# ElesionKyrie/Extreme-Video-Compression-With-Prediction-Using-Pre-trainded-Diffusion-Models-

Measured on AMD Instinct MI355X. Metric: decoded frames/sec (128x128x30) at q3, higher is better.
Workload: dtype f32

## Files before the change

extreme-video-compression-with-prediction-using-pre-trainded-diffusion-models-_amd/csrc/conv_igemm.hip:

```cpp
#include <hip/hip_runtime.h>
#include <stdint.h>
#include <stdio.h>
#include "../../include/evc_hip.h"

typedef float f32x16 __attribute__((ext_vector_type(16)));
typedef __attribute__((address_space(3))) void lds_void;
typedef const __attribute__((address_space(1))) void glb_void;

#ifndef EVC_CONV_TAIL
#define EVC_CONV_TAIL 1
#endif
#ifndef EVC_CONV_TM1
#define EVC_CONV_TM1 1
#endif
#ifndef EVC_SPLIT_WIDE_TILES
#define EVC_SPLIT_WIDE_TILES 1
#endif

#ifndef EVC_SPLIT_INTERLEAVE
#define EVC_SPLIT_INTERLEAVE 5
#endif

namespace {

constexpr int BM_MAX = 128;
constexpr int KC = 16;

constexpr int MODE_PLAIN = 0, MODE_AFFINE = 1, MODE_AFFINE_SILU = 2, MODE_SILU = 3, MODE_RELU = 4;

struct ConvK {
    const float* src0; const float* src1; int C0; int C1; int ld0; int ld1;
    const float* coef_a; const float* coef_s;
    const float* w; const float* bias; const float* res; int ld_res;
    float out_scale; int act_out;
    float* out; int ld_out;
    int B, H, W, Co, CoPad, KH, KW;
    int M, HW, nchunk, nsteps, steps_per_split, splits;
    float* ws;
    float* stats;
    const float* w_hdr;
    const unsigned* in_bound;
    int tail_first, tail_splits, tail_sps, tail_rows;
    int cut_chunk;
    const float* x2_src0; const float* x2_src1; int x2_C0, x2_C1, x2_ld0, x2_ld1;
    const char* x2_w;
    const float* x2_hdr;
    const unsigned* x2_bound;
};

__device__ __forceinline__ float in_scale(const ConvK& p) {
    if (!p.in_bound) return 1.0f;
    const float b = sqrtf(__uint_as_float(*p.in_bound));
    if (!(b < 3.0e38f)) return __builtin_nanf("");
    return b > 0.f ? ldexpf(1.0f, 6 - ilogbf(b)) : 1.0f;
}

__device__ __forceinline__ float silu_f(float v) { return v * __builtin_amdgcn_rcpf(1.0f + __expf(-v)); }

__device__ __forceinline__ float act_fn(float v, int act) {
    if (act == EVC_ACT_SILU) return silu_f(v);
    if (act == EVC_ACT_RELU) return v < 0.f ? 0.f : v;
    return v;
}

template <int MODE>
__device__ __forceinline__ float4 transform(float4 v, const float4& a, const float4& s, bool ok) {
    if (MODE == MODE_AFFINE || MODE == MODE_AFFINE_SILU) {
        v.x = v.x * a.x + s.x; v.y = v.y * a.y + s.y; v.z = v.z * a.z + s.z; v.w = v.w * a.w + s.w;
    }
    if (MODE == MODE_AFFINE_SILU || MODE == MODE_SILU) {
        v.x = silu_f(v.x); v.y = silu_f(v.y); v.z = silu_f(v.z); v.w = silu_f(v.w);
    }
    if (MODE == MODE_RELU) {
        v.x = v.x < 0.f ? 0.f : v.x; v.y = v.y < 0.f ? 0.f : v.y; v.z = v.z < 0.f ? 0.f : v.z; v.w = v.w < 0.f ? 0.f : v.w;
    }
    v.x = ok ? v.x : 0.f; v.y = ok ? v.y : 0.f; v.z = ok ? v.z : 0.f; v.w = ok ? v.w : 0.f;
    return v;
}

template <int TM, int TN>
__device__ __forceinline__ void mfma_group(f32x16 (&acc)[TM][TN], const float4 (&a)[TM], const float4 (&b)[TN]) {
#define EVC_MFMA_E(e)                                                                                   \
    _Pragma("unroll") for (int i = 0; i < TM; ++i) _Pragma("unroll") for (int j = 0; j < TN; ++j)      \
        acc[i][j] = __builtin_amdgcn_mfma_f32_32x32x2f32(a[i].e, b[j].e, acc[i][j], 0, 0, 0);
    EVC_MFMA_E(x) EVC_MFMA_E(y) EVC_MFMA_E(z) EVC_MFMA_E(w)
#undef EVC_MFMA_E
}

template <int TM, int TN, int WM, bool PARTIAL, bool RES, bool STATS, bool ACT>
__device__ __forceinline__ void conv_epilogue_full(const ConvK& p, f32x16 (&acc)[TM][TN], int m0, int n0, int split,
                                                   int wm, int wn, int l31, int half, bool tail) {
    constexpr int BM = 32 * TM * WM;
    const int ws_m0 = tail ? p.tail_first * BM : 0;
    const size_t ws_M = tail ? (size_t)p.tail_rows : (size_t)p.M;
    const float ascale = p.w_hdr ? p.w_hdr[0] / in_scale(p) : 1.0f;
    const float oscale = p.out_scale;
    const int mw = m0 + wm * 32 * TM + 4 * half;
    const int cw = n0 + wn * 32 * TN + l31;
    const bool has_res = RES && (!ACT || p.res != nullptr), has_stats = STATS && (!ACT || p.stats != nullptr);
#pragma unroll
// ... 921 lines not shown
    if (nmac > 0) {
        chunk_setup();
        load_coefs();
        load_a();
        dma_w(0);
        store_a(0);
        if (1 < nst) advance_w();
    }
    __syncthreads();

    int wb = 0, sidx = 0;

    for (int g = 0; g < nmac; ++g) {
        const int ab = g & 1;
        {
            EVC_RR_NEXT_W()
            __builtin_amdgcn_sched_barrier(0);
            if (g + 1 < nmac) advance_l();
            load_a();
            __builtin_amdgcn_sched_barrier(0);
            EVC_RR_FRAGS(0)
            EVC_RR_TERMS(0, SP::NTERM)
            __builtin_amdgcn_sched_barrier(0);
            asm volatile("s_waitcnt vmcnt(2) lgkmcnt(0)\n\ts_barrier" ::: "memory");
            __builtin_amdgcn_sched_barrier(0);
            wb ^= 1; ++sidx;
        }
        {
            EVC_RR_NEXT_W()
            EVC_RR_FRAGS(1)
            EVC_RR_TERMS(0, SP::NTERM)
            __syncthreads();
            wb ^= 1; ++sidx;
        }
        {
            EVC_RR_NEXT_W()
            __builtin_amdgcn_sched_barrier(0);
            EVC_RR_FRAGS(2)
            EVC_RR_TERMS(0, SP::NTERM / 2)
            __builtin_amdgcn_sched_barrier(0);
            store_a(ab ^ 1);
            __builtin_amdgcn_sched_barrier(0);
            EVC_RR_TERMS(SP::NTERM / 2, SP::NTERM)
            __builtin_amdgcn_sched_barrier(0);
            __syncthreads();
            wb ^= 1; ++sidx;
        }
    }
#undef EVC_RR_TERMS
#undef EVC_RR_FRAGS
#undef EVC_RR_NEXT_W

    conv_epilogue<TM, TN, WM>(p, acc, m0, n0, split, wm, wn, l31, half, tail);
}

template <bool PARTIAL, bool RES, bool STATS, bool ACT>
__device__ __forceinline__ void wide_epilogue_t(const ConvK& p, f32x16 (&acc)[4][3], char* lds, int m0, int n0, int split,
                                                int wave, int lane, bool tail) {
    constexpr int TM = 4, TN = 3, BM = 256, RS = 36;
    const int wm = wave >> 1, wn = wave & 1;
    const int l31 = lane & 31, half = lane >> 5;
    const int ws_m0 = tail ? p.tail_first * BM : 0;
    const size_t ws_M = tail ? (size_t)p.tail_rows : (size_t)p.M;
    const float ascale = p.w_hdr[0] / in_scale(p);
    const float oscale = p.out_scale;
    const bool has_res = RES && (!ACT || p.res != nullptr), has_stats = STATS && (!ACT || p.stats != nullptr);
    float* const patch0 = reinterpret_cast<float*>(lds) + wave * 2 * 32 * RS;
    const int wr = lane >> 3, wc = (lane & 7) * 4;
    const int mw = m0 + wm * 32 * TM;
    const int prow = 4 * half * RS + l31;
    constexpr int RD = 4;
    float4 rq[RD][4];
    const auto res_load = [&](int t, float4 (&dst)[4]) {
        const int jj = t / TM, ii = t - jj * TM;
        const float* rp = p.res + (size_t)(mw + ii * 32 + wr) * p.ld_res + n0 + wn * 32 * TN + jj * 32 + wc;
#pragma unroll
        for (int k = 0; k < 4; ++k) dst[k] = *reinterpret_cast<const float4*>(rp + (size_t)(8 * k) * p.ld_res);
    };
    if (has_res) {
#pragma unroll
        for (int t = 0; t < RD - 1; ++t) res_load(t, rq[t]);
    }
#pragma unroll
    for (int j = 0; j < TN; ++j) {
        const int cj = n0 + wn * 32 * TN + j * 32;
        const float bias = (!PARTIAL && p.bias) ? p.bias[cj + l31] : 0.f;
        float4 ssum = make_float4(0.f, 0.f, 0.f, 0.f), ssq = make_float4(0.f, 0.f, 0.f, 0.f);
#pragma unroll
        for (int i = 0; i < TM; ++i) {
            const int mb = mw + i * 32;
            const int tt = j * TM + i;
            if (has_res && tt + RD - 1 < TM * TN) res_load(tt + RD - 1, rq[(tt + RD - 1) % RD]);
            float* const P = patch0 + ((i * TN + j) & 1) * 32 * RS;
#pragma unroll
            for (int r = 0; r < 16; ++r) P[prow + ((r & 3) + 8 * (r >> 2)) * RS] = acc[i][j][r] * ascale + bias;
#pragma unroll
            for (int k = 0; k < 4; ++k) {
                float4 q = *reinterpret_cast<const float4*>(P + (wr + 8 * k) * RS + wc);
                const int m = mb + wr + 8 * k;
                if (!PARTIAL) {
                    if (has_res) { const float4& rr = rq[tt % RD][k]; q.x += rr.x; q.y += rr.y; q.z += rr.z; q.w += rr.w; }
                    q.x *= oscale; q.y *= oscale; q.z *= oscale; q.w *= oscale;
                    if (ACT) { q.x = act_fn(q.x, p.act_out); q.y = act_fn(q.y, p.act_out); q.z = act_fn(q.z, p.act_out); q.w = act_fn(q.w, p.act_out); }
                    if (STATS) {
                        ssum.x += q.x; ssum.y += q.y; ssum.z += q.z; ssum.w += q.w;
                        ssq.x += q.x * q.x; ssq.y += q.y * q.y; ssq.z += q.z * q.z; ssq.w += q.w * q.w;
// ... 571 lines not shown

extern "C" long long evc_conv_packed_bytes(int Co, int Ci, int KH, int KW, int arith) {
    const long long elems = evc_conv_packed_floats(Co, Ci, KH, KW);
    switch (arith) {
        case EVC_ARITH_F32: return elems * 4;
        case EVC_ARITH_BF16X6: return elems * 6;
        case EVC_ARITH_F16X3: return F16_HDR_BYTES + elems * 4;
        default: return EVC_EINVAL;
    }
}

extern "C" int evc_conv_pack_weights(const float* w, void* packed, int Co, int Ci, int KH, int KW, int arith,
                                     void* stream) {
    if (arith == EVC_ARITH_F32) return evc_conv_pack_weights_f32(w, (float*)packed, Co, Ci, KH, KW, stream);
    if (arith != EVC_ARITH_BF16X6 && arith != EVC_ARITH_F16X3) return EVC_EINVAL;
    if (!w || !packed || Co <= 0 || Ci <= 0 || Ci % KC != 0 || KH <= 0 || KW <= 0) return EVC_EINVAL;
    const long long total = evc_conv_packed_floats(Co, Ci, KH, KW);
    int grid = (int)((total + 255) / 256 > 4096 ? 4096 : (total + 255) / 256);
    hipStream_t st = (hipStream_t)stream;
    if (arith == EVC_ARITH_BF16X6) {
        hipLaunchKernelGGL(conv_pack_split_kernel, dim3(grid), dim3(256), 0, st, w, (__bf16*)packed, Co,
                           evc_conv_co_pad(Co), Ci, KH, KW);
    } else {
        if (hipMemsetAsync(packed, 0, F16_HDR_BYTES, st) != hipSuccess) return EVC_ELAUNCH;
        const size_t n = (size_t)Co * Ci * KH * KW;
        hipLaunchKernelGGL(conv_absmax_kernel, dim3(grid), dim3(256), 0, st, w, n, reinterpret_cast<unsigned*>(packed) + 2);
        hipLaunchKernelGGL(conv_pack_f16_kernel, dim3(grid), dim3(256), 0, st, w, (char*)packed, Co,
                           evc_conv_co_pad(Co), Ci, KH, KW);
    }
    return hipGetLastError() == hipSuccess ? EVC_OK : EVC_ELAUNCH;
}

static int conv_validate(const evc_conv_args* a) {
    if (!a || !a->src0 || !a->w_packed || !a->out) return EVC_EINVAL;
    if (a->C0 <= 0 || a->C0 % KC != 0 || a->C1 < 0 || a->C1 % KC != 0) return EVC_EINVAL;
    if (a->C1 > 0 && !a->src1) return EVC_EINVAL;
    if ((a->ld0 != 0 && (a->ld0 < a->C0 || (a->ld0 & 3))) || (a->ld1 != 0 && (a->ld1 < a->C1 || (a->ld1 & 3))))
        return EVC_EINVAL;
    if ((a->coef_a == nullptr) != (a->coef_s == nullptr)) return EVC_EINVAL;
    if (a->B <= 0 || a->H <= 0 || a->W <= 0 || a->Co <= 0) return EVC_EINVAL;
    if (a->KH <= 0 || a->KW <= 0 || !(a->KH & 1) || !(a->KW & 1)) return EVC_EINVAL;
    if (a->ld_out < a->Co || (a->res && a->ld_res < a->Co)) return EVC_EINVAL;
    if ((long long)a->B * a->H * a->W > 0x7fffffffLL) return EVC_EINVAL;
    if (a->arith != EVC_ARITH_F32 && a->arith != EVC_ARITH_BF16X6 && a->arith != EVC_ARITH_F16X3) return EVC_EINVAL;
    if (a->x2_w_packed) {
        if (!a->x2_src0 || !a->x2_bound || a->x2_C0 <= 0 || a->x2_C0 % KC != 0 || a->x2_C1 < 0 || a->x2_C1 % KC != 0) return EVC_EINVAL;
        if (a->x2_C1 > 0 && !a->x2_src1) return EVC_EINVAL;
        if ((a->x2_ld0 != 0 && (a->x2_ld0 < a->x2_C0 || (a->x2_ld0 & 3))) || (a->x2_ld1 != 0 && (a->x2_ld1 < a->x2_C1 || (a->x2_ld1 & 3))))
            return EVC_EINVAL;
    }
    return EVC_OK;
}

struct TileCfg { int tm, tn, bm, bn; long long tiles; int splits; int reuse; int wide; int steps_per_split;
                 int tail_first, tail_tiles, tail_splits, tail_sps;
                 int cut_chunk; };
static int g_wide_cut = 1;
static int g_tail_split = EVC_CONV_TAIL;
static int g_wide_tiles = EVC_SPLIT_WIDE_TILES;
static int g_no_reuse = 0;
static int g_wide_mid = 1;
static int g_wide256 = 1;
static int g_force_tm = 0;

static void split_tile_cfg(const evc_conv_args* a, long long M, long long ntile, int nsteps, TileCfg& c, bool rr_ok) {
    const double K = (double)a->KH * a->KW * (a->C0 + a->C1);
    const bool f16 = a->arith == EVC_ARITH_F16X3 && rr_ok;
    const double E = f16 ? 20.0 : 6.0, F2 = f16 ? 1.5 : 1.0;
    const auto grid_time = [&](long long n, double sps) {
        const long long R = n / 512, rem = n - R * 512;
        return (sps + E) * ((double)R * F2 + (rem == 0 ? 0.0 : (rem <= 256 && f16 ? 1.0 : F2)));
    };
    double best = 1e300;
    int best_tm = 2, best_s = 1;
    c.tail_first = 0; c.tail_tiles = 0; c.tail_splits = 1; c.tail_sps = 0;
    for (int tm = 2; tm >= 1; --tm) {
        if (g_force_tm && tm != g_force_tm) continue;
        const long long tiles = ((M + 64 * tm - 1) / (64 * tm)) * ntile;
        const int smax = a->splits > 0 ? a->splits : (nsteps / 4 < 1 ? 1 : (nsteps / 4 > 32 ? 32 : nsteps / 4));
        for (int s = a->splits > 0 ? a->splits : 1; s <= smax; ++s) {
            const double sps = (double)((nsteps + s - 1) / s);
            const double slab_mb = (double)s * (double)M * a->Co * 4.0 / 1e6;
            const double pen = s > 1 ? 1.0 + (slab_mb > 192.0 ? 300.0 : 40.0) * s / K : 1.0;
            const double tmf = tm == 1 ? (a->KH * a->KW > 1 ? 0.5 / (rr_ok ? 0.55 : 0.75) : 0.5) : 1.0;
            const double t = grid_time(tiles * s, sps) * pen * tmf;
            if (t < best * 0.9999) { best = t; best_tm = tm; best_s = s; }
        }
    }
    c.tm = best_tm;
    c.bm = 64 * c.tm;
    c.tiles = ((M + c.bm - 1) / c.bm) * ntile;
    c.splits = best_s;
    if (rr_ok && g_tail_split && a->splits <= 0 && !g_force_tm && M % 128 == 0) {
        const long long tm_all = M / 128, wgs = tm_all * ntile;
        const long long R = wgs / 512;
        const long long main_m = R * 512 / ntile, tail_m = tm_all - main_m;
        const int unit = 3 * 9;
        if (R >= 1 && tail_m > 0 && nsteps >= 2 * unit) {
            int ts = (int)(512 / (tail_m * ntile));
            if (ts > nsteps / unit) ts = nsteps / unit;
            if (ts >= 2) {
                int sps = (nsteps + ts - 1) / ts;
                sps = (sps + 2) / 3 * 3;
                ts = (nsteps + sps - 1) / sps;
                const double t_tail = grid_time(main_m * ntile, (double)nsteps) +
                                      grid_time(tail_m * ntile * ts, (double)sps) * (1.0 + 40.0 * ts / K);
                if (ts >= 2 && t_tail < best * 0.98) {
                    c.tm = 2; c.bm = 128; c.tiles = wgs; c.splits = 1;
                    c.tail_first = (int)main_m; c.tail_tiles = (int)tail_m; c.tail_splits = ts; c.tail_sps = sps;
                }
            }
        }
    }
}

static inline bool is_split_arith(int arith) { return arith == EVC_ARITH_BF16X6 || arith == EVC_ARITH_F16X3; }
static inline int arith_planes(int arith) { return arith == EVC_ARITH_F16X3 ? 2 : 3; }
constexpr long long LDS_CAP = 160 * 1024;

static long long rr_lds_bytes(int np, int bm, int W, int bn) {
    return (long long)np * 32 * (2LL * (bm / W) * (W + 2) + 2LL * bn);
}

static long long wide_lds_bytes(int W, bool x2) { return (x2 ? 6LL : 4LL) * (256 / W + 2) * (W + 2) * 32; }

static bool wide_ok(const evc_conv_args* a) {
    const bool mode_ok = a->coef_a ? a->act_in == EVC_ACT_SILU : a->act_in == EVC_ACT_NONE;
    return g_wide256 && mode_ok && a->arith == EVC_ARITH_F16X3 && a->KH == 3 && a->KW == 3 && a->Co % 192 == 0 &&
           (a->W == 16 || a->W == 32 || a->W == 64 || a->W == 128) && ((long long)a->H * a->W) % 256 == 0 &&
           a->ld_out % 4 == 0 && (!a->res || a->ld_res % 4 == 0);
}

static TileCfg conv_tile_cfg(const evc_conv_args* a) {
    TileCfg c;
    c.wide = 0;
    c.cut_chunk = 0;
    const long long M = (long long)a->B * a->H * a->W;
    const int CoPad = evc_conv_co_pad(a->Co);
    c.tn = pick_tn(CoPad);
    c.bn = 64 * c.tn;
    const long long ntile = CoPad / c.bn;
    const int nsteps = a->KH * a->KW * ((a->C0 + a->C1) / KC);
    c.reuse = 0;
    if (is_split_arith(a->arith)) {
        const int np = arith_planes(a->arith);
        const bool rr_ok = !g_no_reuse && a->KH == 3 && a->KW == 3 && a->W >= 4 && 128 % a->W == 0 &&
                           rr_lds_bytes(np, 128, a->W, c.bn) <= LDS_CAP;
        split_tile_cfg(a, M, ntile, nsteps, c, rr_ok);
        if (rr_ok && c.tm == 2) c.reuse = 1;
        if (c.reuse && c.splits == 1 && !c.tail_tiles && g_wide_tiles && M % 256 == 0 && rr_lds_bytes(np, 256, a->W, c.bn) <= LDS_CAP) {
            const long long t256 = (M / 256) * ntile;
            if ((t256 >= 512 && t256 % 256 == 0) || t256 >= 6 * 256) {
                c.bm = 256;
                c.tiles = t256;
            }
        }
    } else {
        c.tail_first = 0; c.tail_tiles = 0; c.tail_splits = 1; c.tail_sps = 0;
        c.tm = (!EVC_CONV_TM1 || ((M + 127) / 128) * ntile >= 64) ? 2 : 1;
        if (g_force_tm) c.tm = g_force_tm;
        c.bm = 64 * c.tm;
        c.tiles = ((M + c.bm - 1) / c.bm) * ntile;
        long long splits = 1;
        if (a->splits > 0) splits = a->splits;
        else if (c.tiles < 384) {
            splits = (640 + c.tiles / 2) / c.tiles;
            const int max_by_steps = nsteps / 8 > 0 ? nsteps / 8 : 1;
            if (splits > max_by_steps) splits = max_by_steps;
            if (splits > 32) splits = 32;
            if (splits < 1) splits = 1;
        }
        c.splits = (int)splits;
    }
    if (wide_ok(a) && a->splits <= 0 && !g_force_tm) {
        const long long tm_all = M / 256, nt = a->Co / 192, wgs = tm_all * nt;
        if (wgs >= 256) {
            const int nchunk = (a->C0 + a->C1) / KC;
            c.wide = 1; c.reuse = 0; c.tm = 4; c.tn = 3; c.bm = 256; c.bn = 192; c.tiles = wgs; c.splits = 1;
            c.tail_first = 0; c.tail_tiles = 0; c.tail_splits = 1; c.tail_sps = 0;
            const long long Rr = wgs / 256;
            const long long main_m = Rr * 256 / nt, tail_m = tm_all - main_m;
            if (g_tail_split && tail_m > 0) {
                int ts = (int)(256 / (tail_m * nt));
                if (ts > nchunk / 3) ts = nchunk / 3;
                if (ts >= 2) {
                    const int cps = (nchunk + ts - 1) / ts;
                    ts = (nchunk + cps - 1) / cps;
                    c.tail_first = (int)main_m; c.tail_tiles = (int)tail_m; c.tail_splits = ts; c.tail_sps = cps * 9;
                }
            }
            c.steps_per_split = nsteps;
            return c;
        }
        if (g_wide_mid && wgs >= 32) {
            const int nchunk = (a->C0 + a->C1) / KC;
            int best_s = 0;
            double best_t = 1e300;
            for (int sp = 1; sp <= 8 && wgs * sp <= 256 && nchunk / sp >= 4; ++sp) {
                const int cps = (nchunk + sp - 1) / sp;
                const double slab_mb = sp > 1 ? (double)sp * M * a->Co * 4.0 / 1e6 : 0.0;
                const double t = 23000.0 + 13900.0 * cps + (sp > 1 ? 2.0 * 2000.0 * (5.0 + slab_mb / 4.0) : 0.0);
                if (t < best_t) { best_t = t; best_s = sp; }
            }
            if (best_s > 0 && wgs * best_s >= 128) {
                const int cps = (nchunk + best_s - 1) / best_s;
                c.wide = 1; c.reuse = 0; c.tm = 4; c.tn = 3; c.bm = 256; c.bn = 192; c.tiles = wgs;
                c.tail_first = 0; c.tail_tiles = 0; c.tail_splits = 1; c.tail_sps = 0;
                c.splits = (nchunk + cps - 1) / cps;
                c.steps_per_split = cps * 9;
                if (g_wide_cut && best_s == 1 && wgs > 128 && nchunk >= 6) {
                    const long long idle = 256 - wgs, r = (wgs + idle - 1) / idle;
                    const double slab_mb = 2.0 * M * a->Co * 4.0 / 1e6;
                    const double comb = 2.0 * 2000.0 * (5.0 + slab_mb / 4.0);
                    int cut = 0;
                    double t_cut = best_t * 0.95;
                    for (int sh = 1; sh <= nchunk / 2; ++sh) {
                        const double tl = 23000.0 + 13900.0 * (nchunk - sh), ts = (double)r * (23000.0 + 13900.0 * sh);
                        const double t = (tl > ts ? tl : ts) + comb;
                        if (t < t_cut) { t_cut = t; cut = nchunk - sh; }
                    }
                    if (cut > 0) { c.splits = 2; c.cut_chunk = cut; c.steps_per_split = cut * 9; }
                }
                return c;
            }
        }
    }
    const int unit = c.reuse ? a->KW : 1;
    int sps = (nsteps + c.splits - 1) / c.splits;
    sps = (sps + unit - 1) / unit * unit;
    c.steps_per_split = sps;
    c.splits = (nsteps + sps - 1) / sps;
    return c;
}

extern "C" int evc_conv_set_option(const char* name, int value) {
    if (!name) return EVC_EINVAL;
    const auto is = [&](const char* s) { int i = 0; while (s[i] && s[i] == name[i]) ++i; return s[i] == 0 && name[i] == 0; };
    if (is("wide_tiles")) { g_wide_tiles = value; return EVC_OK; }
    if (is("row_reuse")) { g_no_reuse = !value; return EVC_OK; }
    if (is("tail_split")) { g_tail_split = value; return EVC_OK; }
    if (is("wide256")) { g_wide256 = value; return EVC_OK; }
    if (is("wide_mid")) { g_wide_mid = value; return EVC_OK; }
    if (is("wide_cut")) { g_wide_cut = value; return EVC_OK; }
    return EVC_EINVAL;
}

extern "C" int evc_conv_fused_1x1_supported(const evc_conv_args* a) {
    if (conv_validate(a) != EVC_OK) return 0;
    if (a->arith != EVC_ARITH_F16X3 || a->KH != 3 || a->KW != 3) return 0;
    const TileCfg c = conv_tile_cfg(a);
    return (c.reuse == 1 || c.wide) ? 1 : 0;
}

extern "C" int evc_conv_kernel_name(const evc_conv_args* a, char* buf, int n) {
    if (!buf || n <= 0 || conv_validate(a) != EVC_OK) return EVC_EINVAL;
    int mode;
    if (a->coef_a) mode = a->act_in == EVC_ACT_SILU ? MODE_AFFINE_SILU : MODE_AFFINE;
    else mode = a->act_in == EVC_ACT_SILU ? MODE_SILU : a->act_in == EVC_ACT_RELU ? MODE_RELU : MODE_PLAIN;
    const TileCfg c = conv_tile_cfg(a);
    int len;
    if (c.wide) len = snprintf(buf, n, "conv_wide_kernel<%d, %d, %s>", mode, a->W == 128 ? 4 : 3, a->x2_w_packed ? "true" : "false");
    else if (is_split_arith(a->arith)) {
        const int np = arith_planes(a->arith);
        if (c.reuse) len = snprintf(buf, n, "conv_split_rr_kernel<%d, %d, %d, %d>", np, c.bm == 256 ? 4 : 2, c.tn, mode);
        else if (np == 3) len = snprintf(buf, n, "conv_split_kernel<%d, %d, %d>", c.tm, c.tn, mode);
        else len = snprintf(buf, n, "conv_splitn_kernel<2, %d, %d, %d>", c.tm, c.tn, mode);
    } else len = snprintf(buf, n, "conv_igemm_kernel<%d, %d, %d>", c.tm, c.tn, mode);
    return len;
}

extern "C" int evc_conv_choose_splits(const evc_conv_args* a) {
    if (conv_validate(a) != EVC_OK) return EVC_EINVAL;
    return conv_tile_cfg(a).splits;
}

extern "C" int evc_conv_stats_splits(const evc_conv_args* a) {
    if (conv_validate(a) != EVC_OK) return 0;
    const int HW = a->H * a->W;
    if (HW % 64 != 0) return 0;
    const TileCfg c = conv_tile_cfg(a);
    if (c.splits > 1 || c.wide) return HW / 64;
    const long long M = (long long)a->B * HW;
    const int CoPad = evc_conv_co_pad(a->Co);
    if (M % c.bm != 0 || a->Co != CoPad || a->Co % c.bn != 0) return 0;
    return HW / (32 * c.tm);
}

extern "C" long long evc_conv_workspace_bytes(const evc_conv_args* a) {
    if (conv_validate(a) != EVC_OK) return EVC_EINVAL;
    const TileCfg c = conv_tile_cfg(a);
    if (c.tail_tiles) return (long long)c.tail_splits * c.tail_tiles * c.bm * a->Co * (long long)sizeof(float);
    if (c.splits == 1) return 0;
    return (long long)c.splits * a->B * a->H * a->W * a->Co * (long long)sizeof(float);
}

static int ensure_dynamic_lds(const void* fn, unsigned long long* done_mask, size_t lds) {
    if (lds <= 64 * 1024) return EVC_OK;
    if ((long long)lds > LDS_CAP) return EVC_EUNSUPPORTED;
    int dev = 0;
    if (hipGetDevice(&dev) != hipSuccess) return EVC_ELAUNCH;
    const unsigned long long bit = 1ULL << (dev & 63);
    if (__atomic_load_n(done_mask, __ATOMIC_ACQUIRE) & bit) return EVC_OK;
    if (hipFuncSetAttribute(fn, hipFuncAttributeMaxDynamicSharedMemorySize, (int)LDS_CAP) != hipSuccess) return EVC_ELAUNCH;
    __atomic_fetch_or(done_mask, bit, __ATOMIC_RELEASE);
    return EVC_OK;
}

#ifdef EVC_DEV_FAST
#define EVC_MODE_SWITCH(mode, CALL) CALL(MODE_AFFINE_SILU);
#else
#define EVC_MODE_SWITCH(mode, CALL)                                   \
    switch (mode) {                                                   \
        case MODE_AFFINE: CALL(MODE_AFFINE); break;                   \
        case MODE_AFFINE_SILU: CALL(MODE_AFFINE_SILU); break;         \
// ... 15 lines not shown
static int launch_split3(int mode, dim3 grid, size_t lds, hipStream_t st, const ConvK& k) {
#define EVC_CALL(M) hipLaunchKernelGGL((conv_split_kernel<TM, TN, M>), grid, dim3(256), lds, st, k)
    EVC_MODE_SWITCH(mode, EVC_CALL)
#undef EVC_CALL
    return EVC_OK;
}

template <int TM, int TN>
static int launch_split2(int mode, dim3 grid, size_t lds, hipStream_t st, const ConvK& k) {
#define EVC_CALL(M) hipLaunchKernelGGL((conv_splitn_kernel<2, TM, TN, M>), grid, dim3(256), lds, st, k)
    EVC_MODE_SWITCH(mode, EVC_CALL)
#undef EVC_CALL
    return EVC_OK;
}

template <int NP, int WM, int TN, int MODE>
static int launch_split_rr_one(dim3 grid, size_t lds, hipStream_t st, const ConvK& k) {
    static unsigned long long attr_done = 0;
    const int rc = ensure_dynamic_lds(reinterpret_cast<const void*>(&conv_split_rr_kernel<NP, WM, TN, MODE>), &attr_done, lds);
    if (rc != EVC_OK) return rc;
    hipLaunchKernelGGL((conv_split_rr_kernel<NP, WM, TN, MODE>), grid, dim3(128 * WM), lds, st, k);
    return EVC_OK;
}
template <int NP, int WM, int TN>
static int launch_split_rr(int mode, dim3 grid, size_t lds, hipStream_t st, const ConvK& k) {
    int rc = EVC_OK;
#define EVC_CALL(M) rc = launch_split_rr_one<NP, WM, TN, M>(grid, lds, st, k)
    EVC_MODE_SWITCH(mode, EVC_CALL)
#undef EVC_CALL
    return rc;
}

template <int MODE, int NU, bool X2>
static int launch_wide_one(dim3 grid, size_t lds, hipStream_t st, const ConvK& k) {
    static unsigned long long attr_done = 0;
    const int rc = ensure_dynamic_lds(reinterpret_cast<const void*>(&conv_wide_kernel<MODE, NU, X2>), &attr_done, lds);
    if (rc != EVC_OK) return rc;
    hipLaunchKernelGGL((conv_wide_kernel<MODE, NU, X2>), grid, dim3(256), lds, st, k);
    return EVC_OK;
}
template <int MODE>
static int launch_wide_mode(int nu, bool x2, dim3 grid, size_t lds, hipStream_t st, const ConvK& k) {
    if (nu == 4) return x2 ? launch_wide_one<MODE, 4, true>(grid, lds, st, k) : launch_wide_one<MODE, 4, false>(grid, lds, st, k);
    return x2 ? launch_wide_one<MODE, 3, true>(grid, lds, st, k) : launch_wide_one<MODE, 3, false>(grid, lds, st, k);
}
static int launch_wide(int mode, int nu, bool x2, dim3 grid, size_t lds, hipStream_t st, const ConvK& k) {
#ifdef EVC_DEV_FAST
    return launch_wide_mode<MODE_AFFINE_SILU>(nu, x2, grid, lds, st, k);
#else
    if (mode == MODE_AFFINE_SILU) return launch_wide_mode<MODE_AFFINE_SILU>(nu, x2, grid, lds, st, k);
    if (mode == MODE_PLAIN) return launch_wide_mode<MODE_PLAIN>(nu, x2, grid, lds, st, k);
    return EVC_EUNSUPPORTED;
#endif
}

#define EVC_TN_SWITCH(tn, CALL) ((tn) == 3 ? CALL(3) : (tn) == 2 ? CALL(2) : CALL(1))

static int conv2d_impl(const evc_conv_args* a, float* ws, void* stream, hipEvent_t ev_start, hipEvent_t ev_conv_end);

extern "C" int evc_conv2d_nhwc_f32(const evc_conv_args* a, float* ws, void* stream) {
    return conv2d_impl(a, ws, stream, nullptr, nullptr);
}

extern "C" int evc_conv2d_nhwc_profiled_f32(const evc_conv_args* a, float* ws, void* stream, void* ev_start,
                                            void* ev_conv_end) {
    return conv2d_impl(a, ws, stream, (hipEvent_t)ev_start, (hipEvent_t)ev_conv_end);
}

static int conv2d_impl(const evc_conv_args* a, float* ws, void* stream, hipEvent_t ev_start, hipEvent_t ev_conv_end) {
    int rc = conv_validate(a);
    if (rc != EVC_OK) return rc;
    int mode;
    if (a->coef_a) {
        if (a->act_in == EVC_ACT_SILU) mode = MODE_AFFINE_SILU;
        else if (a->act_in == EVC_ACT_NONE) mode = MODE_AFFINE;
        else return EVC_EUNSUPPORTED;
    } else {
        mode = a->act_in == EVC_ACT_SILU ? MODE_SILU : a->act_in == EVC_ACT_RELU ? MODE_RELU : MODE_PLAIN;
        if (a->act_in != EVC_ACT_NONE && a->act_in != EVC_ACT_SILU && a->act_in != EVC_ACT_RELU) return EVC_EINVAL;
    }
    ConvK k;
    k.src0 = a->src0; k.src1 = a->src1 ? a->src1 : a->src0; k.C0 = a->C0; k.C1 = a->C1;
    k.ld0 = a->ld0 > 0 ? a->ld0 : a->C0; k.ld1 = a->ld1 > 0 ? a->ld1 : (a->C1 > 0 ? a->C1 : k.ld0);
    k.coef_a = a->coef_a; k.coef_s = a->coef_s;
    k.w = a->w_packed; k.bias = a->bias; k.res = a->res; k.ld_res = a->ld_res;
    k.w_hdr = nullptr;
    k.in_bound = nullptr;
    if (a->in_bound) {
        if (a->arith != EVC_ARITH_F16X3) return EVC_EINVAL;
        k.in_bound = a->in_bound;
    }
    if (a->arith == EVC_ARITH_F16X3) {
        k.w_hdr = a->w_packed;
        k.w = reinterpret_cast<const float*>(reinterpret_cast<const char*>(a->w_packed) + F16_HDR_BYTES);
    }
    k.out_scale = a->out_scale; k.act_out = a->act_out; k.out = a->out; k.ld_out = a->ld_out;
    k.B = a->B; k.H = a->H; k.W = a->W; k.Co = a->Co; k.CoPad = evc_conv_co_pad(a->Co);
    k.KH = a->KH; k.KW = a->KW;
    k.M = a->B * a->H * a->W; k.HW = a->H * a->W;
    if ((long long)k.M * k.ld0 * 4 >= (1LL << 32) || (long long)k.M * k.ld1 * 4 >= (1LL << 32)) return EVC_EUNSUPPORTED;
    if (a->KH * a->KW > 32) return EVC_EUNSUPPORTED;
    k.nchunk = (a->C0 + a->C1) / KC;
    k.nsteps = a->KH * a->KW * k.nchunk;
    const TileCfg cfg = conv_tile_cfg(a);
    k.splits = cfg.splits;
    k.steps_per_split = cfg.steps_per_split;
    k.ws = ws;
    if ((k.splits > 1 || cfg.tail_tiles) && !ws) return EVC_EINVAL;
    k.stats = k.splits > 1 ? nullptr : a->stats_out;
    if (a->stats_out && evc_conv_stats_splits(a) == 0) return EVC_EINVAL;
    k.x2_w = nullptr; k.x2_hdr = nullptr; k.x2_bound = nullptr; k.x2_src0 = k.x2_src1 = nullptr;
    k.x2_C0 = k.x2_C1 = k.x2_ld0 = k.x2_ld1 = 0;
    if (a->x2_w_packed) {
        if (a->arith != EVC_ARITH_F16X3 || a->KH != 3 || a->KW != 3 || !(cfg.reuse == 1 || cfg.wide)) return EVC_EUNSUPPORTED;
        k.x2_src0 = a->x2_src0; k.x2_src1 = a->x2_src1 ? a->x2_src1 : a->x2_src0;
        k.x2_C0 = a->x2_C0; k.x2_C1 = a->x2_C1;
        k.x2_ld0 = a->x2_ld0 > 0 ? a->x2_ld0 : a->x2_C0;
        k.x2_ld1 = a->x2_ld1 > 0 ? a->x2_ld1 : (a->x2_C1 > 0 ? a->x2_C1 : k.x2_ld0);
        if ((long long)k.M * k.x2_ld0 * 4 >= (1LL << 32) || (long long)k.M * k.x2_ld1 * 4 >= (1LL << 32)) return EVC_EUNSUPPORTED;
        k.x2_hdr = a->x2_w_packed;
        k.x2_w = reinterpret_cast<const char*>(a->x2_w_packed) + F16_HDR_BYTES;
        k.x2_bound = a->x2_bound;
    }
    k.tail_first = 0x7fffffff; k.tail_splits = 1; k.tail_sps = 0; k.tail_rows = 0;
    k.cut_chunk = cfg.wide ? cfg.cut_chunk : 0;
    if (cfg.tail_tiles) {
        k.tail_first = cfg.tail_first; k.tail_splits = cfg.tail_splits; k.tail_sps = cfg.tail_sps;
        k.tail_rows = cfg.tail_tiles * cfg.bm;
    }

    dim3 grid((k.M + cfg.bm - 1) / cfg.bm, k.CoPad / cfg.bn, k.splits);
    if (cfg.tail_tiles) grid.x = cfg.tail_first + cfg.tail_tiles * cfg.tail_splits;
    hipStream_t st = (hipStream_t)stream;
    if (ev_start && hipEventRecord(ev_start, st) != hipSuccess) return EVC_ELAUNCH;
    if (cfg.wide) {
        rc = launch_wide(mode, a->W == 128 ? 4 : 3, a->x2_w_packed != nullptr, grid, (size_t)wide_lds_bytes(a->W, a->x2_w_packed != nullptr), st, k);
    } else if (is_split_arith(a->arith)) {
        const int np = arith_planes(a->arith);
        if (cfg.reuse) {
            const size_t lds_rr = (size_t)rr_lds_bytes(np, cfg.bm, a->W, cfg.bn);
#define EVC_RR4_3(TN) launch_split_rr<3, 4, TN>(mode, grid, lds_rr, st, k)
#define EVC_RR2_3(TN) launch_split_rr<3, 2, TN>(mode, grid, lds_rr, st, k)
#define EVC_RR4_2(TN) launch_split_rr<2, 4, TN>(mode, grid, lds_rr, st, k)
#define EVC_RR2_2(TN) launch_split_rr<2, 2, TN>(mode, grid, lds_rr, st, k)
            if (np == 3) rc = cfg.bm == 256 ? EVC_TN_SWITCH(cfg.tn, EVC_RR4_3) : EVC_TN_SWITCH(cfg.tn, EVC_RR2_3);
            else rc = cfg.bm == 256 ? EVC_TN_SWITCH(cfg.tn, EVC_RR4_2) : EVC_TN_SWITCH(cfg.tn, EVC_RR2_2);
#undef EVC_RR4_3
#undef EVC_RR2_3
#undef EVC_RR4_2
#undef EVC_RR2_2
        } else {
            const size_t lds = (size_t)2 * np * (cfg.bm + cfg.bn) * 32;
#define EVC_S3_2(TN) launch_split3<2, TN>(mode, grid, lds, st, k)
#define EVC_S3_1(TN) launch_split3<1, TN>(mode, grid, lds, st, k)
#define EVC_S2_2(TN) launch_split2<2, TN>(mode, grid, lds, st, k)
#define EVC_S2_1(TN) launch_split2<1, TN>(mode, grid, lds, st, k)
            if (np == 3) rc = cfg.tm == 2 ? EVC_TN_SWITCH(cfg.tn, EVC_S3_2) : EVC_TN_SWITCH(cfg.tn, EVC_S3_1);
            else rc = cfg.tm == 2 ? EVC_TN_SWITCH(cfg.tn, EVC_S2_2) : EVC_TN_SWITCH(cfg.tn, EVC_S2_1);
#undef EVC_S3_2
#undef EVC_S3_1
#undef EVC_S2_2
#undef EVC_S2_1
        }
    } else {
        const size_t lds = (size_t)2 * (cfg.bm + cfg.bn) * KC * sizeof(float);
#define EVC_F_2(TN) launch_mode<2, TN>(mode, grid, lds, st, k)
#define EVC_F_1(TN) launch_mode<1, TN>(mode, grid, lds, st, k)
        rc = cfg.tm == 2 ? EVC_TN_SWITCH(cfg.tn, EVC_F_2) : EVC_TN_SWITCH(cfg.tn, EVC_F_1);
#undef EVC_F_2
#undef EVC_F_1
    }
    if (rc != EVC_OK) return rc;
    if (hipGetLastError() != hipSuccess) return EVC_ELAUNCH;
    if (ev_conv_end && hipEventRecord(ev_conv_end, st) != hipSuccess) return EVC_ELAUNCH;
    if (k.splits > 1) {
        hipLaunchKernelGGL(conv_splitk_reduce_kernel, dim3((k.M + 63) / 64, (k.Co + 63) / 64), dim3(1024), 0, st, ws,
                           k.splits, k.M, k.Co, a->bias, a->res, a->ld_res, a->out_scale, a->act_out, a->out,
                           a->ld_out, a->stats_out);
        if (hipGetLastError() != hipSuccess) return EVC_ELAUNCH;
    }
    if (cfg.tail_tiles) {
        const size_t m0 = (size_t)cfg.tail_first * cfg.bm;
        hipLaunchKernelGGL(conv_splitk_reduce_kernel, dim3((k.tail_rows + 63) / 64, (k.Co + 63) / 64), dim3(1024), 0, st, ws,
                           k.tail_splits, k.tail_rows, k.Co, a->bias, a->res ? a->res + m0 * a->ld_res : nullptr, a->ld_res,
                           a->out_scale, a->act_out, a->out + m0 * a->ld_out, a->ld_out,
                           a->stats_out ? a->stats_out + (m0 / 64) * k.Co * 2 : nullptr);
        if (hipGetLastError() != hipSuccess) return EVC_ELAUNCH;
    }
    return EVC_OK;
// ... 2 lines not shown
```

Measured before the change: 37.22.

## Add weight-stationary split-K conv kernel for small-spatial 3x3 f16x3 layers

Adds a new conv_ws_kernel for 3x3 convolutions on small images (W of 8 or 16, M up to 2304) with many input channels. Each block covers a variable number of pixels and 64 output channels. It stages the input rows in LDS once per chunk and reuses them across the three horizontal taps, and it splits K across many blocks that write partial sums to the workspace. The goal is better parallelism and less input re-fetching than the reuse tile path on these low-occupancy layers. The cost is more workspace traffic, a heuristic split selection, and four template instantiations per mode.

Result: slower. 36.62 (-1.6%).

```diff
diff --git a/extreme-video-compression-with-prediction-using-pre-trainded-diffusion-models-_amd/csrc/conv_igemm.hip b/extreme-video-compression-with-prediction-using-pre-trainded-diffusion-models-_amd/csrc/conv_igemm.hip
--- a/extreme-video-compression-with-prediction-using-pre-trainded-diffusion-models-_amd/csrc/conv_igemm.hip
+++ b/extreme-video-compression-with-prediction-using-pre-trainded-diffusion-models-_amd/csrc/conv_igemm.hip
@@ -46,6 +46,7 @@
     const char* x2_w;
     const float* x2_hdr;
     const unsigned* x2_bound;
+    int ws_pb;
 };
 
 __device__ __forceinline__ float in_scale(const ConvK& p) {
@@ -1073,6 +1074,274 @@
 #undef EVC_RR_NEXT_W
 
     conv_epilogue<TM, TN, WM>(p, acc, m0, n0, split, wm, wn, l31, half, tail);
+}
+
+constexpr int WS_NT = 512;
+constexpr int WS_NI = 5;
+constexpr int WS_NJ = 3;
+constexpr int WS_PB_MAX = 128 * WS_NI;
+constexpr int WS_PATCH = 32 * 36 * 4;
+
+template <int MODE, bool X2, int NTI>
+__device__ __forceinline__ void conv_ws_body(const ConvK& p, char* smem_b) {
+    typedef Split<2> SP;
+    typedef f16x8 vec;
+    constexpr int RB = 32;
+    constexpr int WBUF = 3 * 2 * 64 * RB;
+    constexpr bool HAS_COEF = MODE == MODE_AFFINE || MODE == MODE_AFFINE_SILU;
+    const int PB = p.ws_pb;
+    const int m0 = blockIdx.x * PB;
+    const int pbc = min(PB, p.M - m0);
+    const int nt32 = pbc >> 5;
+    const int SR = (PB / p.W) * (p.W + 2);
+    const int APL = SR * RB;
+    char* const As = smem_b;
+    char* const Ws = smem_b + 4 * APL;
+
+    const int tid = threadIdx.x;
+    const int lane = tid & 63;
+    const int wave = __builtin_amdgcn_readfirstlane(tid >> 6);
+    const int wm = wave >> 1, wn = wave & 1;
+    const int l31 = lane & 31, half = lane >> 5;
+    const int n0 = blockIdx.y * 64;
+    const int split = blockIdx.z;
+    const int Ct = p.C0 + p.C1;
+    const int kh = tid & 1;
+
+    int it_m[WS_NJ], it_lds[WS_NJ], it_b[WS_NJ];
+    unsigned it_ok[WS_NJ];
+#pragma unroll
+    for (int j = 0; j < WS_NJ; ++j) {
+        const int pl = (tid + WS_NT * j) >> 1;
+        const bool valid = pl < pbc;
+        const int plc = valid ? pl : 0;
+        const int mm = m0 + plc;
+        const int b = mm / p.HW;
+        const int y = (mm - b * p.HW) / p.W;
+        it_m[j] = mm; it_b[j] = b;
+        unsigned ok = valid ? 8u : 0u;
+#pragma unroll
+        for (int ty = 0; ty < 3; ++ty) ok |= ((valid && y + ty - 1 >= 0 && y + ty - 1 < p.H) ? 1u : 0u) << ty;
+        it_ok[j] = ok;
+        const int srow = plc + 2 * (plc / p.W) + 1;
+        it_lds[j] = srow * RB + 16 * (kh ^ ((srow >> 3) & 1));
+    }
+    int abase[NTI];
+#pragma unroll
+    for (int i = 0; i < NTI; ++i) {
+        const int t = wm + 4 * i;
+        const int ml = (t < nt32 ? t : 0) * 32 + l31;
+        abase[i] = ml + 2 * (ml / p.W);
+    }
+    const int w_rd = (wn * 32 + l31) * RB + 16 * (half ^ ((l31 >> 3) & 1));
+
+    const unsigned slab = 2u * (unsigned)p.CoPad * RB;
+    const unsigned w_tap = (unsigned)p.nchunk * slab;
+    const unsigned wsrc = (unsigned)((((wave >> 1) & 1) * p.CoPad + n0 + (wave & 1) * 32) * RB + lane * 16);
+    const int tx_a = wave >> 2;
+    const int wdst_a = ((tx_a * 2 + ((wave >> 1) & 1)) * 64 + (wave & 1) * 32) * RB;
+    const int wdst_b = ((2 * 2 + ((wave >> 1) & 1)) * 64 + (wave & 1) * 32) * RB;
+
+    const int units = p.nchunk * 3;
+    const int ups = p.steps_per_split / 3;
+    const int u_begin = split * ups;
+    const int nmac = max(0, min(units, u_begin + ups) - u_begin);
+    int n2 = 0, c2_begin = 0;
+    float s2 = 1.0f;
+    if (X2) {
+        const int nch2 = (p.x2_C0 + p.x2_C1) / KC;
+        const int per = (nch2 + p.splits - 1) / p.splits;
+        c2_begin = min(nch2, split * per);
+        n2 = min(nch2, c2_begin + per) - c2_begin;
+        const float b = sqrtf(__uint_as_float(*p.x2_bound));
+        if (!(b < 3.0e38f)) s2 = __builtin_nanf("");
+        else if (b > 0.f) s2 = ldexpf(1.0f, 6 - ilogbf(b));
+    }
+    const int total = n2 + nmac;
+    const float xscale = F16_ACT_SCALE * in_scale(p);
+    const float xscale2 = F16_ACT_SCALE * s2;
+
+    float4 areg[WS_NJ][2], ca[WS_NJ][2], cs[WS_NJ][2];
+    auto issue_x2 = [&](int s) {
+        char* wl = Ws + (s & 1) * WBUF;
+        {
+            const int c = c2_begin + s;
+            if (wave >= 4)
+                __builtin_amdgcn_global_load_lds((glb_void*)(p.x2_w + (unsigned)c * slab + wsrc), (lds_void*)(wl + wdst_a), 16, 0, 0);
+            const int cc = c * KC;
+            const bool first = cc < p.x2_C0;
+            const char* src = reinterpret_cast<const char*>(first ? p.x2_src0 : p.x2_src1);
+            const unsigned ld = (unsigned)(first ? p.x2_ld0 : p.x2_ld1);
+            const unsigned co = (unsigned)(first ? cc : cc - p.x2_C0) + 8u * kh;
+#pragma unroll
+            for (int j = 0; j < WS_NJ; ++j) {
+                const unsigned o = ((unsigned)it_m[j] * ld + co) * 4u;
+                areg[j][0] = *reinterpret_cast<const float4*>(src + o);
+                areg[j][1] = *reinterpret_cast<const float4*>(src + o + 16);
+            }
+        }
+    };
+    auto issue = [&](int s) {
+        char* wl = Ws + (s & 1) * WBUF;
+        {
+            const int u = u_begin + (s - n2);
+            const int chunk = u / 3, ty = u - chunk * 3;
+            const char* wt = reinterpret_cast<const char*>(p.w) + (unsigned)(ty * 3 * p.nchunk + chunk) * slab + wsrc;
+            __builtin_amdgcn_global_load_lds((glb_void*)(wt + (unsigned)tx_a * w_tap), (lds_void*)(wl + wdst_a), 16, 0, 0);
+            if (wave < 4)
+                __builtin_amdgcn_global_load_lds((glb_void*)(wt + 2u * w_tap), (lds_void*)(wl + wdst_b), 16, 0, 0);
+            const int c = chunk * KC;
+            const bool first = c < p.C0;
+            const char* src = reinterpret_cast<const char*>(first ? p.src0 : p.src1);
+            const unsigned ld = (unsigned)(first ? p.ld0 : p.ld1);
+            const unsigned co = (unsigned)(first ? c : c - p.C0) + 8u * kh;
+            if (HAS_COEF && (ty == 0 || s == n2)) {
+#pragma unroll
+                for (int j = 0; j < WS_NJ; ++j) {
+                    const size_t o = (size_t)it_b[j] * Ct + c + 8 * kh;
+                    ca[j][0] = *reinterpret_cast<const float4*>(p.coef_a + o);
+                    ca[j][1] = *reinterpret_cast<const float4*>(p.coef_a + o + 4);
+                    cs[j][0] = *reinterpret_cast<const float4*>(p.coef_s + o);
+                    cs[j][1] = *reinterpret_cast<const float4*>(p.coef_s + o + 4);
+                }
+            }
+#pragma unroll
+            for (int j = 0; j < WS_NJ; ++j) {
+                const bool ok = (it_ok[j] >> ty) & 1u;
+                const unsigned o = ((unsigned)(it_m[j] + (ok ? (ty - 1) * p.W : 0)) * ld + co) * 4u;
+                areg[j][0] = *reinterpret_cast<const float4*>(src + o);
+                areg[j][1] = *reinterpret_cast<const float4*>(src + o + 16);
+            }
+        }
+    };
+    auto commit_x2 = [&](int s) {
+        char* A = As + (s & 1) * 2 * APL;
+#pragma unroll
+        for (int j = 0; j < WS_NJ; ++j) {
+            if (!(it_ok[j] & 8u)) continue;
+            vec pl[2];
+            SP::split(areg[j][0], areg[j][1], xscale2, pl);
+            *reinterpret_cast<vec*>(A + it_lds[j]) = pl[0];
+            *reinterpret_cast<vec*>(A + APL + it_lds[j]) = pl[1];
+        }
+    };
+    auto commit = [&](int s) {
+        char* A = As + (s & 1) * 2 * APL;
+        const int u = u_begin + (s - n2);
+        const int ty = u - (u / 3) * 3;
+#pragma unroll
+        for (int j = 0; j < WS_NJ; ++j) {
+            if (!(it_ok[j] & 8u)) continue;
+            vec pl[2];
+            const bool ok = (it_ok[j] >> ty) & 1u;
+            SP::split(transform<MODE>(areg[j][0], ca[j][0], cs[j][0], ok), transform<MODE>(areg[j][1], ca[j][1], cs[j][1], ok), xscale, pl);
+            *reinterpret_cast<vec*>(A + it_lds[j]) = pl[0];
+            *reinterpret_cast<vec*>(A + APL + it_lds[j]) = pl[1];
+        }
+    };
+
+    f32x16 acc[NTI];
+#pragma unroll
+    for (int i = 0; i < NTI; ++i)
+#pragma unroll
+        for (int r = 0; r < 16; ++r) acc[i][r] = 0.f;
+
+    auto tap = [&](int s, int tx) {
+        const char* Ab = As + (s & 1) * 2 * APL;
+        const char* Wb = Ws + (s & 1) * WBUF + tx * (2 * 64 * RB) + w_rd;
+        vec b[2];
+        b[0] = *reinterpret_cast<const vec*>(Wb);
+        b[1] = *reinterpret_cast<const vec*>(Wb + 64 * RB);
+#pragma unroll
+        for (int i0 = 0; i0 < NTI; i0 += 2) {
+            constexpr int NPAIR = 2;
+            vec a[NPAIR][2];
+#pragma unroll
+            for (int d = 0; d < NPAIR; ++d) {
+                if (i0 + d < NTI) {
+                    const int sr = abase[i0 + d] + tx;
+                    const int o = sr * RB + 16 * (half ^ ((sr >> 3) & 1));
+                    a[d][0] = *reinterpret_cast<const vec*>(Ab + o);
+                    a[d][1] = *reinterpret_cast<const vec*>(Ab + APL + o);
+                }
+            }
+#pragma unroll
+            for (int t = 0; t < SP::NTERM; ++t)
+#pragma unroll
+                for (int d = 0; d < NPAIR; ++d)
+                    if (i0 + d < NTI) acc[i0 + d] = SP::mfma(a[d][SP::qa(t)], b[SP::qb(t)], acc[i0 + d]);
+        }
+    };
+
+    for (int o = tid * 16; o < 4 * APL; o += WS_NT * 16) *reinterpret_cast<float4*>(As + o) = make_float4(0.f, 0.f, 0.f, 0.f);
+    __syncthreads();
+    if (X2 && n2 > 0) { issue_x2(0); commit_x2(0); }
+    else if (nmac > 0) { issue(n2); commit(n2); }
+    asm volatile("s_waitcnt vmcnt(0)" ::: "memory");
+    __syncthreads();
+
+    if (X2) {
+        for (int s = 0; s < n2; ++s) {
+            const bool nx = s + 1 < n2, nm = !nx && nmac > 0;
+            if (nx) issue_x2(s + 1);
+            else if (nm) issue(s + 1);
+            tap(s, 1);
+            if (nx) commit_x2(s + 1);
+            else if (nm) commit(s + 1);
+            asm volatile("s_waitcnt vmcnt(0)" ::: "memory");
+            __syncthreads();
+        }
+        if (n2 > 0) {
+            const float r = (p.x2_hdr[0] / s2) / (p.w_hdr[0] / in_scale(p));
+#pragma unroll
+            for (int i = 0; i < NTI; ++i)
+#pragma unroll
+                for (int e = 0; e < 16; ++e) acc[i][e] *= r;
+        }
+    }
+    for (int s = n2; s < total; ++s) {
+        if (s + 1 < total) issue(s + 1);
+        tap(s, 0);
+        if (s + 1 < total) commit(s + 1);
+        tap(s, 1);
+        tap(s, 2);
+        asm volatile("s_waitcnt vmcnt(0)" ::: "memory");
+        __syncthreads();
+    }
+
+    const float ascale = p.w_hdr[0] / in_scale(p);
+    float* const patch = reinterpret_cast<float*>(smem_b + wave * WS_PATCH);
+#pragma unroll
+    for (int i = 0; i < NTI; ++i) {
+        const int t = wm + 4 * i;
+        if (t >= nt32) break;
+#pragma unroll
+        for (int r = 0; r < 16; ++r) patch[((r & 3) + 8 * (r >> 2) + 4 * half) * 36 + l31] = acc[i][r] * ascale;
+        __builtin_amdgcn_fence(__ATOMIC_RELEASE, "wavefront");
+        __builtin_amdgcn_wave_barrier();
+        __builtin_amdgcn_fence(__ATOMIC_ACQUIRE, "wavefront");
+        float* o = p.ws + ((size_t)split * p.M + (m0 + t * 32)) * p.Co + n0 + wn * 32;
+#pragma unroll
+        for (int k = 0; k < 4; ++k) {
+            const int row = (lane >> 3) + 8 * k, c4 = (lane & 7) * 4;
+            *reinterpret_cast<float4*>(o + (size_t)row * p.Co + c4) = *reinterpret_cast<const float4*>(patch + row * 36 + c4);
+        }
+        __builtin_amdgcn_fence(__ATOMIC_RELEASE, "wavefront");
+        __builtin_amdgcn_wave_barrier();
+        __builtin_amdgcn_fence(__ATOMIC_ACQUIRE, "wavefront");
+    }
+}
+
+template <int MODE, bool X2>
+__global__ __launch_bounds__(WS_NT, 1) void conv_ws_kernel(ConvK p) {
+    extern __shared__ __attribute__((aligned(16))) char smem_b[];
+    const int wm = __builtin_amdgcn_readfirstlane((int)threadIdx.x >> 7);
+    const int nt32 = min(p.ws_pb, p.M - (int)blockIdx.x * p.ws_pb) >> 5;
+    const int nti = (nt32 - wm + 3) >> 2;
+    if (nti >= 5) conv_ws_body<MODE, X2, 5>(p, smem_b);
+    else if (nti == 4) conv_ws_body<MODE, X2, 4>(p, smem_b);
+    else if (nti == 3) conv_ws_body<MODE, X2, 3>(p, smem_b);
+    else conv_ws_body<MODE, X2, 2>(p, smem_b);
 }
 
 template <bool PARTIAL, bool RES, bool STATS, bool ACT>
@@ -1750,7 +2019,7 @@
     return EVC_OK;
 }
 
-struct TileCfg { int tm, tn, bm, bn; long long tiles; int splits; int reuse; int wide; int steps_per_split;
+struct TileCfg { int tm, tn, bm, bn; long long tiles; int splits; int reuse; int wide; int ws; int steps_per_split;
                  int tail_first, tail_tiles, tail_splits, tail_sps;
                  int cut_chunk; };
 static int g_wide_cut = 1;
@@ -1759,6 +2028,7 @@
 static int g_no_reuse = 0;
 static int g_wide_mid = 1;
 static int g_wide256 = 1;
+static int g_small_ws = 1;
 static int g_force_tm = 0;
 
 static void split_tile_cfg(const evc_conv_args* a, long long M, long long ntile, int nsteps, TileCfg& c, bool rr_ok) {
@@ -1829,9 +2099,43 @@
            a->ld_out % 4 == 0 && (!a->res || a->ld_res % 4 == 0);
 }
 
+static long long ws_lds_bytes(int pb, int W) {
+    const long long k = 4LL * (pb / W) * (W + 2) * 32 + 2LL * 3 * 2 * 64 * 32;
+    return k > 8LL * WS_PATCH ? k : 8LL * WS_PATCH;
+}
+
+static bool ws_cfg(const evc_conv_args* a, long long M, TileCfg& c) {
+    const bool mode_ok = a->coef_a ? a->act_in == EVC_ACT_SILU : a->act_in == EVC_ACT_NONE;
+    const int nchunk = (a->C0 + a->C1) / KC;
+    if (!g_small_ws || !mode_ok || a->arith != EVC_ARITH_F16X3 || a->KH != 3 || a->KW != 3 || (a->W != 8 && a->W != 16) ||
+        a->splits > 0 || g_force_tm || a->Co % 64 != 0 || M % 32 != 0 || M < 320 || M > 2304 || nchunk < 24)
+        return false;
+    long long nblk = (M + 575) / 576;
+    const int pb = (int)(((M + nblk - 1) / nblk + 31) / 32 * 32);
+    nblk = (M + pb - 1) / pb;
+    if (M - (nblk - 1) * pb < 128 || pb > WS_PB_MAX || ws_lds_bytes(pb, a->W) > LDS_CAP) return false;
+    const int ntile = a->Co / 64, units = nchunk * 3;
+    const int smax = (int)(256 / (nblk * ntile));
+    int best_s = 0;
+    double best_t = 1e300;
+    for (int s = 2; s <= smax && units / s >= 3; ++s) {
+        const int ups = (units + s - 1) / s;
+        const double t = 1.25 * ups + (double)s * (double)M * a->Co * 4.0 / 4.0e6;
+        if (t < best_t) { best_t = t; best_s = s; }
+    }
+    if (best_s < 2) return false;
+    const int ups = (units + best_s - 1) / best_s;
+    c.ws = 1; c.reuse = 0; c.wide = 0; c.tm = 2; c.tn = 1; c.bm = pb; c.bn = 64; c.tiles = nblk * ntile;
+    c.splits = (units + ups - 1) / ups;
+    c.steps_per_split = ups * 3;
+    c.tail_first = 0; c.tail_tiles = 0; c.tail_splits = 1; c.tail_sps = 0;
+    return c.splits >= 2;
+}
+
 static TileCfg conv_tile_cfg(const evc_conv_args* a) {
     TileCfg c;
     c.wide = 0;
+    c.ws = 0;
     c.cut_chunk = 0;
     const long long M = (long long)a->B * a->H * a->W;
     const int CoPad = evc_conv_co_pad(a->Co);
@@ -1923,6 +2227,7 @@
             }
         }
     }
+    if (c.reuse && c.bm == 128 && c.splits > 1 && !c.tail_tiles && ws_cfg(a, M, c)) return c;
     const int unit = c.reuse ? a->KW : 1;
     int sps = (nsteps + c.splits - 1) / c.splits;
     sps = (sps + unit - 1) / unit * unit;
@@ -1940,6 +2245,7 @@
     if (is("wide256")) { g_wide256 = value; return EVC_OK; }
     if (is("wide_mid")) { g_wide_mid = value; return EVC_OK; }
     if (is("wide_cut")) { g_wide_cut = value; return EVC_OK; }
+    if (is("small_ws")) { g_small_ws = value; return EVC_OK; }
     return EVC_EINVAL;
 }
 
@@ -1947,7 +2253,7 @@
     if (conv_validate(a) != EVC_OK) return 0;
     if (a->arith != EVC_ARITH_F16X3 || a->KH != 3 || a->KW != 3) return 0;
     const TileCfg c = conv_tile_cfg(a);
-    return (c.reuse == 1 || c.wide) ? 1 : 0;
+    return (c.reuse == 1 || c.wide || c.ws) ? 1 : 0;
 }
 
 extern "C" int evc_conv_kernel_name(const evc_conv_args* a, char* buf, int n) {
@@ -1958,6 +2264,7 @@
     const TileCfg c = conv_tile_cfg(a);
     int len;
     if (c.wide) len = snprintf(buf, n, "conv_wide_kernel<%d, %d, %s>", mode, a->W == 128 ? 4 : 3, a->x2_w_packed ? "true" : "false");
+    else if (c.ws) len = snprintf(buf, n, "conv_ws_kernel<%d, %s>", mode, a->x2_w_packed ? "true" : "false");
     else if (is_split_arith(a->arith)) {
         const int np = arith_planes(a->arith);
         if (c.reuse) len = snprintf(buf, n, "conv_split_rr_kernel<%d, %d, %d, %d>", np, c.bm == 256 ? 4 : 2, c.tn, mode);
@@ -2079,6 +2386,22 @@
     if (mode == MODE_PLAIN) return launch_wide_mode<MODE_PLAIN>(nu, x2, grid, lds, st, k);
     return EVC_EUNSUPPORTED;
 #endif
+}
+
+template <int MODE, bool X2>
+static int launch_ws_one(dim3 grid, size_t lds, hipStream_t st, const ConvK& k) {
+    static unsigned long long attr_done = 0;
+    const int rc = ensure_dynamic_lds(reinterpret_cast<const void*>(&conv_ws_kernel<MODE, X2>), &attr_done, lds);
+    if (rc != EVC_OK) return rc;
+    hipLaunchKernelGGL((conv_ws_kernel<MODE, X2>), grid, dim3(WS_NT), lds, st, k);
+    return EVC_OK;
+}
+static int launch_ws(int mode, bool x2, dim3 grid, size_t lds, hipStream_t st, const ConvK& k) {
+    if (mode == MODE_AFFINE_SILU) return x2 ? launch_ws_one<MODE_AFFINE_SILU, true>(grid, lds, st, k) : launch_ws_one<MODE_AFFINE_SILU, false>(grid, lds, st, k);
+#ifndef EVC_DEV_FAST
+    if (mode == MODE_PLAIN) return x2 ? launch_ws_one<MODE_PLAIN, true>(grid, lds, st, k) : launch_ws_one<MODE_PLAIN, false>(grid, lds, st, k);
+#endif
+    return EVC_EUNSUPPORTED;
 }
 
 #define EVC_TN_SWITCH(tn, CALL) ((tn) == 3 ? CALL(3) : (tn) == 2 ? CALL(2) : CALL(1))
@@ -2139,7 +2462,7 @@
     k.x2_w = nullptr; k.x2_hdr = nullptr; k.x2_bound = nullptr; k.x2_src0 = k.x2_src1 = nullptr;
     k.x2_C0 = k.x2_C1 = k.x2_ld0 = k.x2_ld1 = 0;
     if (a->x2_w_packed) {
-        if (a->arith != EVC_ARITH_F16X3 || a->KH != 3 || a->KW != 3 || !(cfg.reuse == 1 || cfg.wide)) return EVC_EUNSUPPORTED;
+        if (a->arith != EVC_ARITH_F16X3 || a->KH != 3 || a->KW != 3 || !(cfg.reuse == 1 || cfg.wide || cfg.ws)) return EVC_EUNSUPPORTED;
         k.x2_src0 = a->x2_src0; k.x2_src1 = a->x2_src1 ? a->x2_src1 : a->x2_src0;
         k.x2_C0 = a->x2_C0; k.x2_C1 = a->x2_C1;
         k.x2_ld0 = a->x2_ld0 > 0 ? a->x2_ld0 : a->x2_C0;
@@ -2151,6 +2474,7 @@
     }
     k.tail_first = 0x7fffffff; k.tail_splits = 1; k.tail_sps = 0; k.tail_rows = 0;
     k.cut_chunk = cfg.wide ? cfg.cut_chunk : 0;
+    k.ws_pb = cfg.ws ? cfg.bm : 0;
     if (cfg.tail_tiles) {
         k.tail_first = cfg.tail_first; k.tail_splits = cfg.tail_splits; k.tail_sps = cfg.tail_sps;
         k.tail_rows = cfg.tail_tiles * cfg.bm;
@@ -2162,6 +2486,8 @@
     if (ev_start && hipEventRecord(ev_start, st) != hipSuccess) return EVC_ELAUNCH;
     if (cfg.wide) {
         rc = launch_wide(mode, a->W == 128 ? 4 : 3, a->x2_w_packed != nullptr, grid, (size_t)wide_lds_bytes(a->W, a->x2_w_packed != nullptr), st, k);
+    } else if (cfg.ws) {
+        rc = launch_ws(mode, a->x2_w_packed != nullptr, grid, (size_t)ws_lds_bytes(cfg.bm, a->W), st, k);
     } else if (is_split_arith(a->arith)) {
         const int np = arith_planes(a->arith);
         if (cfg.reuse) {
```
